# hzxie/Stereo-3D-Reconstruction

Measured on AMD Instinct MI355X. Metric: stereo pairs/s forward (batch 32, 224x224 -> 32^3 voxel), higher is better.
Workload: dtype f32

## Files before the change

stereo-3d-reconstruction_amd/csrc/s3r_api.hip:

```cpp
#include "s3r_host.h"

#include <algorithm>
#include <cmath>
#include <cstdio>
#include <cstring>
#include <utility>

using namespace s3rh;

namespace {

inline bool misaligned16(const void* p) { return ((uintptr_t)p & 15) != 0; }
int bf16_align_fail(const char* what, const void* p) {
    return fail(S3R_ERR_INVALID, "%s must be 16-byte aligned (got %p): bf16 tensors are accessed 16 bytes at a time", what, p);
}

struct ConvCall {
    const s3r_conv_desc* d;
    Geo g;
    const void* x; const void* x2; int nsplit, x_u8;
    const void* w; const float* scale; const float* shift;
    void* y;
    float* scratch; int64_t scratch_elems;
    hipStream_t s;
// ... 274 lines not shown
        return fail(S3R_ERR_INVALID, "a consumer's operand is written from the class-parallel launch form of a 3D two-axis layer only (the semi-fused "
                    "form of this batch keeps the plain output: s3r_chain_forward plans that itself)");
    if (g2.bmax <= 0 || ((pre || to_v || p.out_mode) && g2.bmax < d->batch))
        return fail(S3R_ERR_INVALID, "two-axis Winograd form: the transformed input of this batch exceeds 2 GiB (at most %d samples per "
                    "call with a producer-written input: s3r_conv_wino_input_elems)", g2.bmax);
    int rc = check_scratch(c, need.total, "the two-axis Winograd form of this layer needs");
    if (rc) return rc;
    p.w = c.wf() + packed_layout(d, g).wino2;
    p.x = pre ? c.xf() : c.scratch;
    p.part = c.scratch + need.v;
    p.Nd = g2.sg; p.Nh = g2.sg; p.Nw = g2.out;
    p.kd = 1; p.kh = 1; p.kw = g2.kw; p.T = g2.kw;
    p.x_hs = g2.wp; p.x_ds = g2.sg * g2.wp; p.x_cs = g2.sg * g2.sg * g2.wp;
    p.x_org = 0;
    set_divs(p);
    if (g2.ax == 2) {
        p.Nd = 1; p.Nw = g2.sg;
        p.dS = s3r::FastDiv((unsigned)(g2.sg * g2.sg));
        p.dW = s3r::FastDiv((unsigned)g2.sg);
    }
    p.Hout = g2.out; p.Dout = g2.out;
    p.ncls = g2.ncls;
    p.ksplit = 1;
    const int64_t x_sample = g.x_elems / d->batch;
    ps.launches = 0;
    for (int b0 = 0; b0 < d->batch; b0 += g2.bmax) {
        const int nb = sub_batch(d->batch, b0, g2.bmax);
        hipError_t e = hipSuccess;
        if (!pre) {
            s3r::AuxScope aux(c.s, 4.0 * ((double)nb * x_sample + (double)(g2.ax == 2 ? g2.ncls * d->cin * s3r::wino2_npad(g2.pos_sample * nb) : g2.v_sample * nb)));
            if (g2.ax == 2)
                e = s3r::launch_wino2p_input(c.xf() + (int64_t)b0 * x_sample, c.scratch, nb, d->cin, g2.wp, g2.wp, g2.sg, g2.sg,
                                             s3r::wino2_npad(g2.pos_sample * nb), c.s);
            else
                e = s3r::launch_wino2_input(c.xf() + (int64_t)b0 * x_sample, c.scratch, g2.ax, (long long)nb * d->cin, g2.wp, g2.wp, g2.wp, g2.sg,
                                            g2.sg, c.s);
            if (e != hipSuccess) return hip_fail(e, "two-axis Winograd input transform launch");
            ps.launches += 1;
        }
        set_sub_batch(p, c.yf(), b0, nb, g2.v_sample);
        p.x_cls = nb * d->cin * p.x_cs;
        int nl = 0;
        e = s3r::launch_conv_wino2(p, g2.ax, wino2_form_of(d, p.Ntotal, form), to_v, c.s, &nl);
        if (e != hipSuccess) return hip_fail(e, "two-axis Winograd conv launch");
        ps.launches += nl;
    }
// ... 1202 lines not shown
```

stereo-3d-reconstruction_amd/csrc/s3r_conv_wino.hip:

```cpp
#include "s3r_kernels.h"
#include <cstdlib>

namespace s3r {

typedef float wf32x16 __attribute__((ext_vector_type(16)));
typedef float wv2f __attribute__((ext_vector_type(2)));
template <int N> struct WVec;
template <> struct WVec<1> { typedef float type; };
template <> struct WVec<2> { typedef wv2f type; };
typedef float wv4f __attribute__((ext_vector_type(4)));
template <> struct WVec<4> { typedef wv4f type; };
template <int N>
__device__ __forceinline__ float wvget(const typename WVec<N>::type& v, int i) {
    if constexpr (N == 1) return v; else return v[i];
}

#define S3R_LDS_PTR_W(p) ((__attribute__((address_space(3))) void*)(p))

#ifndef S3R_WNB
#define S3R_WNB 2
#endif
#ifndef S3R_WBK
#define S3R_WBK 32
#endif
// ... 190 lines not shown
        y[3] = fmaf(8.f, d34, d12) + m[5];
    } else {
        const float t00 = m[0] + m[1], t01 = m[1] - m[2];
        const float t10 = m[3] + m[4], t11 = m[4] - m[5];
        const float t20 = m[6] + m[7], t21 = m[7] - m[8];
        y[0] = t00 + t10;
        y[1] = t01 + t11;
        y[2] = t10 - t20;
        y[3] = t11 - t21;
    }
}
template <int KIND>
__device__ __forceinline__ int wino_out_off(int i, int y_ds, int y_hs) {
    if constexpr (KIND == 1) return i * y_hs;
    else return (i >> 1) * 2 * y_ds + (i & 1) * 2 * y_hs;
}
__device__ __forceinline__ float wino_act(float y, float sc, float sf, float lo) { return fmaxf(fmaf(y, sc, sf), lo); }
__device__ __forceinline__ float wino_head_act(float t, int act) {
    if (act == ACT_RELU) return fmaxf(t, 0.f);
    if (act == ACT_SIGMOID) return __builtin_amdgcn_rcpf(1.f + __expf(-t));
    return t;
}

template <int VEC, int KIND, int WN, bool CP, bool HEAD, bool XM = false, bool SEMI = false>
__device__ __forceinline__ void wino_body(const ConvParams& p, const int bid_in, const int nwg_in, const int n_begin,
                                          const int n_end, float* __restrict__ wsmem) {
    constexpr bool DECONV = KIND == 2;
    constexpr int NCLS = WinoKind<KIND>::NCLS, R = WinoKind<KIND>::R;
    constexpr int WM = 4 / WN, TM = 2 / WM, BN = 32 * WN;
    constexpr int NACC = CP ? 1 : NCLS;
    static_assert(KIND == 1 || KIND == 2, "F(4,3) convolution or F(2,2) transposed convolution");
    static_assert(!SEMI || (KIND == 1 && !CP && !HEAD), "the semi-fused form: serial F(4,3) row classes of one depth class");
    static_assert(WN == 4 || WN == 2, "4 waves as 1 x 4 or 2 x 2");
    static_assert(!HEAD || (DECONV && !CP && WN == 2), "the fused head: serial transposed form");
    float* As = wsmem;
    constexpr int BSTG = (DECONV ? 2 : 1) * WBK * BN;
    float* Bs = wsmem + WNB * WBK * WBM;
    constexpr int PB = 64 * VEC;
    constexpr int NPIECE_B = WBK * BN / PB;
    static_assert(NPIECE_B % 4 == 0, "B pieces divide over the 4 waves");
    constexpr int NPB = NPIECE_B / 4;
    constexpr bool B_WIDE = BN >= PB;
    constexpr int PPR = B_WIDE ? BN / PB : 1;
    constexpr int RPP = B_WIDE ? 1 : PB / BN;
    constexpr int LPR_B = BN / VEC;
    constexpr int NPD = WNPA + NPB;

    const int tid = threadIdx.x;
    const int lane = tid & 63;
    const int wave = __builtin_amdgcn_readfirstlane(tid >> 6);
    const int wm = wave / WN, wn = wave % WN;
    const int j = lane & 31, h = lane >> 5;
#ifdef S3R_ABLATE
    unsigned long long tl0 = 0, tl1 = 0, tl2 = 0;
    if (p.debug == 7) tl0 = __builtin_amdgcn_s_memrealtime();
#endif

// ... 4 lines not shown
        const int q = nwg >> 3, r = nwg & 7, xcd = bid & 7, slot = bid >> 3;
        const int item = (xcd < r ? xcd * (q + 1) : r * (q + 1) + (xcd - r) * q) + slot;
        const int ntile = p.m_tiles * n_tiles;
        const int c = item / ntile;
        bid = item - c * ntile;
        if constexpr (DECONV) { pc = c / NCLS; cls0 = c - pc * NCLS; } else cls0 = SEMI ? c * NCLS : c;
    } else if constexpr (DECONV) {
        const int nwg = nwg_in >> 3;
        const int item = (bid & 7) * nwg + (bid >> 3);
        bid = item >> 3;
        pc = item & 7;
    } else {
        const int nwg = nwg_in;
        const int q = nwg >> 3, r = nwg & 7, xcd = bid & 7, slot = bid >> 3;
        bid = (xcd < r ? xcd * (q + 1) : r * (q + 1) + (xcd - r) * q) + slot;
    }
    const int rd = (pc >> 2) & 1, rh = (pc >> 1) & 1, rw = pc & 1;
    const int m_tile = bid % p.m_tiles, n_tile = bid / p.m_tiles;
    const int m0 = m_tile * WBM, n0 = n_begin + n_tile * BN;
    const int S = p.Nd * p.Nh * p.Nw;
    const int T = DECONV ? 2 : p.T;
    const int chunks = p.Cin / WBK;
    const int nkt = T * chunks;
    const int total = NACC * nkt;

    int bvoff;
    {
        int col, lrow;
        if (B_WIDE) { col = (wave % PPR) * PB + lane * VEC; lrow = 0; }
        else        { col = (lane % LPR_B) * VEC;           lrow = lane / LPR_B; }
        int n = n0 + col;
        if (n >= n_end) n = n_end - VEC;
        const int b = p.dS.div(n);
        int rem = n - b * S;
        const int pd = p.dHW.div(rem);
        rem -= pd * p.Nh * p.Nw;
        const int q = p.dW.div(rem);
        const int pw = rem - q * p.Nw;
        if constexpr (DECONV)
            bvoff = (b * p.Cin * p.x_cs + (2 * pd + rd) * p.x_ds + (2 * q + rh) * p.x_hs + pw + rw + lrow * p.x_cs) * 4;
        else
            bvoff = (b * p.Cin * p.x_cs + p.x_org + pd * p.x_ds + q * p.x_hs + pw + lrow * p.x_cs) * 4;
    }
    const int avoff = ((lane >> 4) * p.CoutPad + (lane & 15) * 4) * 4;
    const __amdgpu_buffer_rsrc_t xrsrc =
        __builtin_amdgcn_make_buffer_rsrc(const_cast<float*>(p.x), 0, (int)p.x_bytes, 0x00020000);
    const __amdgpu_buffer_rsrc_t drsrc =
        __builtin_amdgcn_make_buffer_rsrc(const_cast<float*>(DECONV ? p.xd : p.x), 0, (int)p.x_bytes, 0x00020000);
    const size_t x_el = (size_t)p.x_bytes / 4;
    const __amdgpu_buffer_rsrc_t wrsrc = __builtin_amdgcn_make_buffer_rsrc(
        const_cast<float*>(p.w), 0,
        (int)((unsigned)(DECONV ? 72 : (p.ncls ? p.ncls : NCLS)) * (unsigned)T * (unsigned)p.Cin * (unsigned)p.CoutPad * 4u),
        0x00020000);
    const int b_row0 = B_WIDE ? wave / PPR : wave * RPP;
    constexpr int B_ROW_STEP = B_WIDE ? 4 / PPR : 4 * RPP;
    const int b_lds0 = B_WIDE ? b_row0 * BN + (wave % PPR) * PB : wave * PB;
    constexpr int B_LDS_STEP = B_WIDE ? B_ROW_STEP * BN : 4 * PB;
    const int cs4 = p.x_cs * 4;

    int c_cls = cls0, c_cc = 0, c_td = 0, c_tw = 0, c_tap = 0;
    int c_kt = (DECONV ? pc * NCLS + cls0 : cls0) * nkt;
    int c_a = cls0 / 3, c_b = cls0 - 3 * (cls0 / 3);
#ifdef S3R_ABLATE
    bool abl_loop = false;
#endif
    auto issue = [&](int buf) __attribute__((always_inline)) {
#ifdef S3R_ABLATE
        const bool skip_a = abl_loop && (p.debug == 3 || p.debug == 5);
        const bool skip_b = abl_loop && (p.debug == 3 || p.debug == 4 || (p.debug == 6 && (DECONV ? c_tap != 0 : c_tw != 0)));
#else
        constexpr bool skip_a = false, skip_b = false;
#endif
        if (!skip_a) {
#pragma unroll
            for (int q = 0; q < WNPA; ++q)
                wdma<16>(wrsrc, As + buf * WBK * WBM + (wave + 4 * q) * 256, avoff,
                         (c_kt * WBK * p.CoutPad + m0) * 4 + (wave + 4 * q) * 4 * p.CoutPad * 4);
        }
        float* sb = Bs + buf * BSTG + b_lds0;
        if constexpr (DECONV) {
            const int b_base = ((c_cc * WBK + b_row0) * p.x_cs + (c_a ? p.x_ds : 0) + (c_b ? p.x_hs : 0) + c_tap) * 4;
            if (skip_b) {
            } else if constexpr (XM) {
                const int t_idx = (c_a != 1 ? 2 : 0) + (c_b != 1 ? 1 : 0);
                const float* tb = t_idx == 0 ? p.x : p.xd + (size_t)(t_idx - 1) * x_el;
                const __amdgpu_buffer_rsrc_t trsrc = __builtin_amdgcn_make_buffer_rsrc(const_cast<float*>(tb), 0, (int)p.x_bytes, 0x00020000);
#pragma unroll
                for (int q = 0; q < NPB; ++q) wdma<4 * VEC>(trsrc, sb + q * B_LDS_STEP, bvoff, b_base + q * B_ROW_STEP * cs4);
            } else if (c_b == 1) {
#pragma unroll
                for (int q = 0; q < NPB; ++q) wdma<4 * VEC>(xrsrc, sb + q * B_LDS_STEP, bvoff, b_base + q * B_ROW_STEP * cs4);
                if (c_a != 1) {
#pragma unroll
                    for (int q = 0; q < NPB; ++q)
                        wdma<4 * VEC>(xrsrc, sb + WBK * BN + q * B_LDS_STEP, bvoff, b_base + p.x_ds * 4 + q * B_ROW_STEP * cs4);
                }
            } else {
#pragma unroll
                for (int q = 0; q < NPB; ++q) wdma<4 * VEC>(drsrc, sb + q * B_LDS_STEP, bvoff, b_base + q * B_ROW_STEP * cs4);
                if (c_a != 1) {
#pragma unroll
                    for (int q = 0; q < NPB; ++q)
                        wdma<4 * VEC>(drsrc, sb + WBK * BN + q * B_LDS_STEP, bvoff, b_base + p.x_ds * 4 + q * B_ROW_STEP * cs4);
                }
            }
            ++c_kt;
            if (++c_tap == 2) {
                c_tap = 0;
                if (++c_cc == chunks) {
                    c_cc = 0; ++c_cls;
                    if (++c_b == 3) { c_b = 0; ++c_a; }
                }
            }
        } else {
            const int b_base = (c_cls * p.x_cls + (c_cc * WBK + b_row0) * p.x_cs + c_td * p.x_ds + c_tw) * 4;
            if (!skip_b) {
#pragma unroll
                for (int q = 0; q < NPB; ++q) wdma<4 * VEC>(xrsrc, sb + q * B_LDS_STEP, bvoff, b_base + q * B_ROW_STEP * cs4);
            }
            ++c_kt;
            if (++c_tw == p.kw) { c_tw = 0; ++c_td; }
            if (++c_tap == T) {
                c_tap = 0; c_td = 0; c_tw = 0;
                if (++c_cc == chunks) { c_cc = 0; ++c_cls; }
            }
        }
    };

    wf32x16 acc[NACC][TM];
#pragma unroll
    for (int c = 0; c < NACC; ++c)
#pragma unroll
        for (int t = 0; t < TM; ++t)
#pragma unroll
            for (int r = 0; r < 16; ++r) acc[c][t][r] = 0.f;

#pragma unroll
    for (int i = 0; i < WNB - 1; ++i)
        if (i < total) issue(i);
    if (total >= WNB - 1) asm volatile("s_waitcnt vmcnt(%0)" :: "n"((WNB - 2) * NPD) : "memory");
    else asm volatile("s_waitcnt vmcnt(0)" ::: "memory");
    __builtin_amdgcn_s_barrier();
    asm volatile("" ::: "memory");
#ifdef S3R_ABLATE
    abl_loop = true;
    if (p.debug == 7) tl1 = __builtin_amdgcn_s_memrealtime();
#endif

    const int a_off = h * WBM + wm * TM * 32 + j * TM;
    const int b_off = h * BN + wn * 32 + j;
    typedef typename WVec<TM>::type AV;
    int cur = 0, g = 0;
    auto run_class = [&](wf32x16 (&ac)[TM], const bool diff) __attribute__((always_inline)) {
        for (int kt = 0; kt < nkt; ++kt, ++g) {
            const bool more = g + WNB - 1 < total;
            if (more) issue(cur == 0 ? WNB - 1 : cur - 1);
            const float* a = As + cur * WBK * WBM + a_off;
            const float* b = Bs + cur * BSTG + b_off;
            if (DECONV && diff) {
#pragma unroll
                for (int ks = 0; ks < WBK / 2; ++ks) {
                    const AV av = *reinterpret_cast<const AV*>(a + ks * 2 * WBM);
                    const float bv = b[ks * 2 * BN] - b[WBK * BN + ks * 2 * BN];
#pragma unroll
                    for (int t = 0; t < TM; ++t) ac[t] = __builtin_amdgcn_mfma_f32_32x32x2f32(wvget<TM>(av, t), bv, ac[t], 0, 0, 0);
                }
            } else {
#pragma unroll
                for (int ks = 0; ks < WBK / 2; ++ks) {
                    const AV av = *reinterpret_cast<const AV*>(a + ks * 2 * WBM);
                    const float bv = b[ks * 2 * BN];
#pragma unroll
                    for (int t = 0; t < TM; ++t) ac[t] = __builtin_amdgcn_mfma_f32_32x32x2f32(wvget<TM>(av, t), bv, ac[t], 0, 0, 0);
                }
            }
            if (more) asm volatile("s_waitcnt vmcnt(%0)" :: "n"((WNB - 2) * NPD) : "memory");
            else asm volatile("s_waitcnt vmcnt(0)" ::: "memory");
// ... 153 lines not shown
                    const float sc = ep_sc[mbase + dm], sf = ep_sf[mbase + dm];
                    float m[NCLS], y[R];
#pragma unroll
                    for (int c = 0; c < NCLS; ++c) m[c] = acc[c][tm][r];
                    wino_out<KIND>(m, y);
                    const int so = dm * row_bytes;
                    if (ok) {
#pragma unroll
                        for (int i = 0; i < R; ++i)
                            if (i < row1) {
                                const float v = wino_act(y[i], sc, sf, lo);
                                __builtin_amdgcn_raw_buffer_store_b32(__builtin_bit_cast(unsigned, v), yrsrc,
                                                                      yvo0 + 4 * wino_out_off<KIND>(i, p.y_ds, p.y_hs), so, 0);
                            }
                    }
                    if ((r & 3) == 3) __builtin_amdgcn_sched_barrier(0);
                }
        }
        S3R_TL_FINISH();
    }
}
#undef S3R_TL_FINISH

template <int VEC, int KIND, int WN, bool CP, bool HEAD, bool XM = false, bool SEMI = false>
__global__ __launch_bounds__(256, (CP || KIND == 1 ? 4 : 3)) void wino_kernel(const ConvParams p) {
    extern __shared__ __attribute__((aligned(16))) float wsmem[];
    wino_body<VEC, KIND, WN, CP, HEAD, XM, SEMI>(p, blockIdx.x, gridDim.x, p.n_begin, p.n_end, wsmem);
}

template <int VEC, int KIND, bool HEAD = false, bool XM = false>
__global__ __launch_bounds__(256, (KIND == 1 ? 4 : 3)) void wino_dual_kernel(const ConvParams p) {
    extern __shared__ __attribute__((aligned(16))) float wsmem[];
    if ((int)blockIdx.x < p.big_wgs)
        wino_body<VEC, KIND, 2, false, HEAD, XM>(p, blockIdx.x, p.big_wgs, p.n_begin, p.n_cut, wsmem);
    else
        wino_body<VEC, KIND, 2, true, false, XM>(p, (int)blockIdx.x - p.big_wgs, (int)gridDim.x - p.big_wgs, p.n_cut, p.n_end, wsmem);
}

template <int KIND, bool HEAD>
__global__ __launch_bounds__(256) void wino_finish_kernel(const ConvParams p, const int n_begin, const int n_end, const int npad) {
    constexpr bool DECONV = KIND == 2;
    constexpr int NCLS = WinoKind<KIND>::NCLS, R = WinoKind<KIND>::R;
    const int S = p.Nd * p.Nh * p.Nw;
    const int nn = n_end - n_begin;
    const int pc = DECONV ? (int)blockIdx.y : 0;
    const int rd = (pc >> 2) & 1, rh = (pc >> 1) & 1, rw = pc & 1;
    const float lo = p.act == ACT_RELU ? 0.f : -__builtin_inff();
    constexpr int NBLK = DECONV ? 8 * NCLS : NCLS;
    const int ntl = npad >> 6;
    const float* __restrict__ base = p.part + (size_t)pc * NCLS * 64;
// ... 326 lines not shown
hipError_t launch_pack_wino2(const float* w, float* wp, int ax, int Cin, int Cout, int CoutPad, hipStream_t s) {
    if (ax == 0) hipLaunchKernelGGL(pack_wino2_kernel<0>, dim3(1024), dim3(256), 0, s, w, wp, Cin, Cout, CoutPad);
    else if (ax == 1) hipLaunchKernelGGL(pack_wino2_kernel<1>, dim3(1024), dim3(256), 0, s, w, wp, Cin, Cout, CoutPad);
    else if (ax == 2) hipLaunchKernelGGL(pack_wino2p_kernel, dim3(1024), dim3(256), 0, s, w, wp, Cin, Cout, CoutPad);
    else return hipErrorInvalidValue;
    return hipGetLastError();
}

__device__ __forceinline__ void wino2_copy_out(const float* __restrict__ lds, float* __restrict__ dst, int count, int tid) {
    if ((count & 3) == 0 && (reinterpret_cast<size_t>(dst) & 15) == 0) {
        for (int i = tid * 4; i < count; i += 1024) *reinterpret_cast<wv4f*>(dst + i) = *reinterpret_cast<const wv4f*>(lds + i);
    } else {
        for (int i = tid; i < count; i += 256) dst[i] = lds[i];
    }
}
__device__ __forceinline__ void wino2_zero_out(float* __restrict__ dst, int count, int tid) {
    if ((count & 3) == 0 && (reinterpret_cast<size_t>(dst) & 15) == 0) {
        for (int i = tid * 4; i < count; i += 1024) *reinterpret_cast<wv4f*>(dst + i) = wv4f{0.f, 0.f, 0.f, 0.f};
    } else {
        for (int i = tid; i < count; i += 256) dst[i] = 0.f;
    }
}

__global__ __launch_bounds__(256) void wino2s_finish_kernel(const ConvParams p, const int npad, const int halo, const int SUB,
                                                            const FastDiv dNd, const FastDiv dMS) {
    constexpr int N = 6, M = 4;
    extern __shared__ __attribute__((aligned(16))) float fsm[];
    const int tid = threadIdx.x;
    const int G = p.Nh * p.Nw, Wp = p.y_hs, slice = p.y_ds, MS = M * slice;
    const float lo = p.act == ACT_RELU ? 0.f : -__builtin_inff();
    const int per_c = p.B * p.Nd;
    const int nrg = (per_c + SUB - 1) / SUB;
    const bool vec = (slice & 3) == 0 && (reinterpret_cast<size_t>(p.y) & 15) == 0;
    for (int item = blockIdx.x; item < p.Cout * nrg; item += gridDim.x) {
        const int mrow = item / nrg;
        const int r0 = (item - mrow * nrg) * SUB;
        const int nsub = per_c - r0 < SUB ? per_c - r0 : SUB;
        for (int i = tid; i < nsub * MS; i += 256) fsm[i] = 0.f;
        __syncthreads();
        const float sc = p.scale ? p.scale[mrow] : 1.f, sf = p.shift ? p.shift[mrow] : 0.f;
        for (int t = tid; t < nsub * G; t += 256) {
            const int sub = p.dHW.div(t);
            const int g = t - sub * G;
            const int sh = p.dW.div(g);
            const int pw = g - sh * p.Nw;
            const int r = r0 + sub;
            const int sd = r - dNd.div(r) * p.Nd;
            const int n = r0 * G + t;
            const float* __restrict__ src = p.part + ((size_t)mrow * (npad >> 6) + (n >> 6)) * (N * M * 64) + (n & 63);
            float* __restrict__ o = fsm + sub * MS + (halo + M * sh) * Wp + halo + pw;
#pragma unroll
            for (int v = 0; v < M; ++v) {
                float m[N], y[M];
#pragma unroll
                for (int a = 0; a < N; ++a) m[a] = src[(a * M + v) * 64];
                wax_at<0>(m, y);
#pragma unroll
                for (int u = 0; u < M; ++u)
                    if (M * sd + u < p.Dout && M * sh + v < p.Hout) o[u * slice + v * Wp] = wino_act(y[u], sc, sf, lo);
            }
        }
        __syncthreads();
        float* __restrict__ yc = p.y + (size_t)mrow * p.y_cs;
        for (int e = vec ? tid * 4 : tid; e < nsub * MS; e += vec ? 1024 : 256) {
            const int sub = dMS.div(e);
            const int off = e - sub * MS;
            const int r = r0 + sub;
            const int b = dNd.div(r);
// ... 10 lines not shown
                const int b = dNd.div(r);
                const int sd = r - b * p.Nd;
                if (sd == 0) wino2_zero_out(yc + (size_t)b * p.y_bs, halo * slice, tid);
                if (sd == p.Nd - 1) wino2_zero_out(yc + (size_t)b * p.y_bs + (size_t)(halo + p.Dout) * slice, halo * slice, tid);
            }
        __syncthreads();
    }
}

template <int AX>
__global__ __launch_bounds__(256) void wino2_finish_flat_kernel(const ConvParams p, const int npad) {
    constexpr int N = WAxis<AX>::N, M = WAxis<AX>::M;
    const int S = p.Nd * p.Nh * p.Nw;
    const int nn = p.Ntotal;
    const float lo = p.act == ACT_RELU ? 0.f : -__builtin_inff();
    const long long total = (long long)p.Cout * nn;
    for (long long i = (long long)blockIdx.x * 256 + threadIdx.x; i < total; i += (long long)gridDim.x * 256) {
        const int mrow = (int)(i / nn);
        const int n = (int)(i - (long long)mrow * nn);
        const int b = p.dS.div(n);
        int rem = n - b * S;
        const int sd = p.dHW.div(rem);
        rem -= sd * p.Nh * p.Nw;
        const int sh = p.dW.div(rem);
        const int pw = rem - sh * p.Nw;
        const float* __restrict__ src = p.part + ((size_t)mrow * (npad >> 6) + (n >> 6)) * (N * N * 64) + (n & 63);
        float t[N][M];
#pragma unroll
        for (int a = 0; a < N; ++a) {
            float m[N], y[M];
#pragma unroll
            for (int c = 0; c < N; ++c) m[c] = src[(a * N + c) * 64];
            wax_at<AX>(m, y);
#pragma unroll
            for (int v = 0; v < M; ++v) t[a][v] = y[v];
        }
        const float sc = p.scale ? p.scale[mrow] : 1.f, sf = p.shift ? p.shift[mrow] : 0.f;
        float* __restrict__ yo = p.y + (size_t)b * p.y_bs + (size_t)mrow * p.y_cs + p.y_org + (size_t)M * sd * p.y_ds + M * sh * p.y_hs + pw;
#pragma unroll
        for (int v = 0; v < M; ++v) {
            float m[N], y[M];
#pragma unroll
            for (int a = 0; a < N; ++a) m[a] = t[a][v];
            wax_at<AX>(m, y);
#pragma unroll
            for (int u = 0; u < M; ++u)
                if (M * sd + u < p.Dout && M * sh + v < p.Hout) yo[(size_t)u * p.y_ds + v * p.y_hs] = wino_act(y[u], sc, sf, lo);
        }
// ... 222 lines not shown
    const int S = p.Nd * p.Nh * p.Nw;
    const int G1 = PROD == 2 ? 8 * S : S;
    const int G2 = CONS == 2 ? vol : SG * SG * Op;
    const int ncb = (p.Cout + CB - 1) / CB;
    const float lo = p.act == ACT_RELU ? 0.f : -__builtin_inff();
    const bool vec2 = CONS == 2 && (Op & 1) == 0 && (reinterpret_cast<size_t>(p.y) & 7) == 0;
    for (int item = blockIdx.x; item < p.B * ncb; item += gridDim.x) {
        const int b = item / ncb;
        const int c0 = (item - b * ncb) * CB;
        const int nc = p.Cout - c0 < CB ? p.Cout - c0 : CB;
        for (int i = tid; i < nc * vol; i += 256) hsm[i] = 0.f;
        __syncthreads();
        for (int t = tid; t < nc * G1; t += 256) {
            const int cl = dG1.div(t);
            int g = t - cl * G1;
            const int mrow = c0 + cl;
            const float sc = p.scale ? p.scale[mrow] : 1.f, sf = p.shift ? p.shift[mrow] : 0.f;
            float* __restrict__ o = hsm + cl * vol + org;
            if constexpr (PROD <= 1) {
                constexpr int N = WAxis<PROD>::N, M = WAxis<PROD>::M;
                const int n = b * S + g;
                const int sd = p.dHW.div(g);
                g -= sd * p.Nh * p.Nw;
                const int sh = p.dW.div(g);
                const int pw = g - sh * p.Nw;
                const float* __restrict__ src = p.part + ((size_t)mrow * (npad >> 6) + (n >> 6)) * (N * N * 64) + (n & 63);
                float tt[N][M];
#pragma unroll
                for (int a = 0; a < N; ++a) {
                    float m[N], y[M];
#pragma unroll
                    for (int c = 0; c < N; ++c) m[c] = src[(a * N + c) * 64];
                    wax_at<PROD>(m, y);
#pragma unroll
                    for (int v = 0; v < M; ++v) tt[a][v] = y[v];
                }
                o += M * sd * ds + M * sh * hs + pw;
#pragma unroll
                for (int v = 0; v < M; ++v) {
                    float m[N], y[M];
#pragma unroll
                    for (int a = 0; a < N; ++a) m[a] = tt[a][v];
                    wax_at<PROD>(m, y);
#pragma unroll
                    for (int u = 0; u < M; ++u)
                        if (M * sd + u < p.Dout && M * sh + v < p.Hout) o[u * ds + v * hs] = wino_act(y[u], sc, sf, lo);
                }
            } else if constexpr (PROD == 2) {
// ... 196 lines not shown
        q.dS = q.dHW = q.dW = FastDiv((unsigned)npad);
        q.kd = q.kh = q.kw = 1; q.T = 1;
        q.x_org = 0; q.x_ds = 0; q.x_hs = 0; q.x_cs = npad; q.x_cls = p.Cin * npad;
        q.x_bytes = (unsigned)(4ull * 36 * p.Cin * npad);
        q.Ntotal = npad; q.n_end = npad;
        const dim3 grid(p.m_tiles * n_tiles * (form == 1 ? 6 : 36));
        if (form == 1) hipLaunchKernelGGL((wino_kernel<4, 1, 2, false, false, false, true>), grid, dim3(256), lds, stream, q);
        else hipLaunchKernelGGL((wino_kernel<4, 1, 2, true, false>), grid, dim3(256), lds, stream, q);
        hipError_t e = hipGetLastError();
        if (e != hipSuccess) return e;
        const long long items = (long long)p.Cout * ((p.B + PL - 1) / PL);
        const dim3 fgrid((unsigned)(items < 16384 ? items : 16384));
        const size_t flds = (size_t)PL * plane * 4;
        AuxScope aux(stream, 4.0 * (double)p.Cout * ((double)(form == 1 ? 24 : 36) * npad + (to_v ? 36.0 * npad : (double)p.B * plane)));
        if (to_v) {
            if (form == 1) hipLaunchKernelGGL((wino2p_finish_kernel<true, true>), fgrid, dim3(256), flds, stream, p, npad, halo, PL);
            else hipLaunchKernelGGL((wino2p_finish_kernel<false, true>), fgrid, dim3(256), flds, stream, p, npad, halo, PL);
        } else if (form == 1) hipLaunchKernelGGL((wino2p_finish_kernel<true, false>), fgrid, dim3(256), flds, stream, p, npad, halo, PL);
        else hipLaunchKernelGGL((wino2p_finish_kernel<false, false>), fgrid, dim3(256), flds, stream, p, npad, halo, PL);
        if (launches) *launches = 2;
        return hipGetLastError();
    }
    if (p.y_ds != p.y_hs * p.y_hs || p.y_cs != (p.Dout + 2 * halo) * p.y_ds) return hipErrorInvalidValue;
    if (form == 1) {
        const int M = wino2_outputs(ax), G = p.Nh * p.Nw;
        if (ax != 0 || (size_t)M * p.y_ds * 4 > 64 * 1024) return hipErrorInvalidValue;
        int SUB = 256 / G < 1 ? 1 : 256 / G;
        if (SUB > p.B * p.Nd) SUB = p.B * p.Nd;
        while (SUB > 1 && (size_t)SUB * M * p.y_ds * 4 > 64 * 1024) --SUB;
        const size_t flds = (size_t)SUB * M * p.y_ds * 4;
        const FastDiv dNd((unsigned)p.Nd), dMS((unsigned)(M * p.y_ds));
        const long long items = (long long)p.Cout * ((p.B * p.Nd + SUB - 1) / SUB);
        const dim3 fgrid((unsigned)(items < 32768 ? items : 32768));
        const dim3 grid(p.m_tiles * n_tiles * 6);
        if (p.Nw % 4 == 0) hipLaunchKernelGGL((wino_kernel<4, 1, 2, false, false, false, true>), grid, dim3(256), lds, stream, p);
        else hipLaunchKernelGGL((wino_kernel<1, 1, 2, false, false, false, true>), grid, dim3(256), lds, stream, p);
        hipError_t e = hipGetLastError();
        if (e != hipSuccess) return e;
        AuxScope aux(stream, 4.0 * (double)p.Cout * (24.0 * n_tiles * WCN + (double)p.B * p.y_cs));
        hipLaunchKernelGGL(wino2s_finish_kernel, fgrid, dim3(256), flds, stream, p, n_tiles * WCN, halo, SUB, dNd, dMS);
        if (launches) *launches = 2;
        return hipGetLastError();
    }
    const dim3 grid(p.m_tiles * n_tiles * p.ncls);
    if (p.Nw % 4 == 0) hipLaunchKernelGGL((wino_kernel<4, 1, 2, true, false>), grid, dim3(256), lds, stream, p);
    else hipLaunchKernelGGL((wino_kernel<1, 1, 2, true, false>), grid, dim3(256), lds, stream, p);
    hipError_t e = hipGetLastError();
    if (e != hipSuccess) return e;
    if (launches) *launches = 2;
    if (p.out_mode) return launch_wino_handoff(p, ax, p.out_mode - 1, n_tiles * WCN, stream);
    const long long total = (long long)p.Cout * p.Ntotal;
    const long long blocks = (total + 255) / 256;
    const dim3 flat((unsigned)(blocks < 8192 ? blocks : 8192));
    AuxScope aux(stream, 4.0 * (double)p.Cout * ((double)p.ncls * n_tiles * WCN + (double)p.B * p.Dout * p.Hout * p.Nw));
    if (ax == 0) hipLaunchKernelGGL(wino2_finish_flat_kernel<0>, flat, dim3(256), 0, stream, p, n_tiles * WCN);
    else hipLaunchKernelGGL(wino2_finish_flat_kernel<1>, flat, dim3(256), 0, stream, p, n_tiles * WCN);
    if (launches) *launches = 2;
    return hipGetLastError();
}

#ifdef S3R_ABLATE
}
extern "C" int s3r_debug_read_timeline_wino(unsigned long long* out, int nblocks) {
    if (nblocks > 65536) nblocks = 65536;
    return hipMemcpyFromSymbol(out, HIP_SYMBOL(s3r::s3r_wino_timeline), sizeof(unsigned long long) * 6 * (size_t)nblocks) == hipSuccess ? nblocks : -1;
}
extern "C" int s3r_debug_clear_timeline_wino() {
    void* ptr = nullptr;
    if (hipGetSymbolAddress(&ptr, HIP_SYMBOL(s3r::s3r_wino_timeline)) != hipSuccess) return -1;
// ... 7 lines not shown
```

stereo-3d-reconstruction_amd/csrc/s3r_kernels.h:

```cpp
#pragma once
#include <hip/hip_runtime.h>
#include <stdint.h>
#include <atomic>

struct s3r_optim_tensor;
struct s3r_augment_desc;

namespace s3r {

struct LdsAttr {
    std::atomic<unsigned long long> done{0};
    hipError_t ensure(const void* fn, int bytes) {
        int dev = 0;
        hipError_t e = hipGetDevice(&dev);
        if (e != hipSuccess) return e;
        if (dev >= 0 && dev < 64 && ((done.load(std::memory_order_relaxed) >> dev) & 1ull)) return hipSuccess;
        e = hipFuncSetAttribute(fn, hipFuncAttributeMaxDynamicSharedMemorySize, bytes);
        if (e == hipSuccess && dev >= 0 && dev < 64) done.fetch_or(1ull << dev, std::memory_order_relaxed);
        return e;
    }
};

inline int cu_count() {
    static std::atomic<int> cached[64];
// ... 58 lines not shown
    int y_step;
    int shuf_s, shuf_nd;
    FastDiv dSC, dS1;
    unsigned x_bytes;
    unsigned y_bytes;
    int transposed;
    int act;
    float slope;
    int Ntotal;
    int n_begin, n_end;
    int n_tiles, m_tiles;
    int n_cut, big_wgs;
    int ksplit;
    float* part;
    int debug;
    const float* head_w;
    const float* head_scale;
    const float* head_shift;
    int head_act;
    int x_cls, Hout, Dout, ncls;
    const float* xd;
    int xd_mode;
    int out_mode;
};

struct TClsEntry {
    int Nd, Nh, Nw, kd, kh, kw, T, x_org, y_org, Ntotal, wg_begin, w_off;
    FastDiv dS, dHW, dW;
};
constexpr int kTClsMax = 27;
struct TClsTable { int n; TClsEntry e[kTClsMax]; };
hipError_t launch_conv_tcls(const ConvParams& base, TClsTable tab, hipStream_t stream);

enum { WINO_SERIAL = 0, WINO_CP = 1, WINO_DUAL = 2 };
struct WinoLaunch { int mode, n_cut; };

struct ConvParamsH {
    const void* x;
    const void* w;
    const float* scale;
    const float* shift;
    void* y;
    float* part;
    int B, Cin, Cout, CoutPad;
    int Nd, Nh, Nw;
    FastDiv dS, dHW, dW, dDH, dH;
// ... 190 lines not shown
```

stereo-3d-reconstruction_amd/csrc/s3r_pointwise.hip:

```cpp
#include "s3r_kernels.h"

namespace s3r {

typedef float v4f __attribute__((ext_vector_type(4)));

__device__ __forceinline__ float apply_act(float v, int act) {
    if (act == ACT_RELU) return fmaxf(v, 0.f);
    if (act == ACT_SIGMOID) return 1.f / (1.f + __expf(-v));
    return v;
}

template <typename TI>
__global__ __launch_bounds__(256) void stem_kernel(const TI* __restrict__ x, const TI* __restrict__ x2, int nsplit,
                                                   const float* __restrict__ wt,
                                                   const float* __restrict__ scale, const float* __restrict__ shift,
                                                   float* __restrict__ y, int N, int Hi, int Wi, int Ho, int Wo,
                                                   int y_cs, int y_hs, int y_org) {
    const int HWo = Ho * Wo;
    const long long total = (long long)N * HWo;
    const long long gid = (long long)blockIdx.x * 256 + threadIdx.x;
    if (gid >= total) return;
    const int n = (int)(gid / HWo);
    const int sp = (int)(gid - (long long)n * HWo);
    const int oh = sp / Wo, ow = sp - oh * Wo;
// ... 300 lines not shown
    float* sl = cvw2_smem;
    float* sr = cvw2_smem + HW;
    const int bc = blockIdx.x;
    const int b = bc / C, c = bc - b * C;
    const float* __restrict__ pl = fl + (size_t)bc * HW;
    const float* __restrict__ pr = fr + (size_t)bc * HW;
    for (int i = threadIdx.x; i < HW; i += 256) {
        sl[i] = pl[i];
        sr[i] = pr[i];
    }
    __syncthreads();
    const int Wp = W + 2, SH = H / 4, SD = (D + 3) / 4;
    const int ds = SH * Wp;
    const int run = SD * ds;
    const int ny = (int)gridDim.y, pph = ny > 1 ? ny / 2 : 1;
    const int half0 = ny > 1 ? (int)blockIdx.y / pph : 0, half1 = ny > 1 ? half0 + 1 : 2;
    const int part = ny > 1 ? (int)blockIdx.y - half0 * pph : 0;
    const int e0 = (part * SD / pph) * ds, e1 = ((part + 1) * SD / pph) * ds;
    for (int half = half0; half < half1; ++half) {
        float* __restrict__ o = V + ((size_t)b * 2 * C + half * C + c) * run;
        for (int e = e0 + threadIdx.x; e < e1; e += 256) {
            const int sd = dPlane.div(e);
            const int rem = e - sd * ds;
            const int sh = dRow.div(rem);
            const int wp = rem - sh * Wp;
            const int w = wp - 1;
            float t[6][6];
#pragma unroll
            for (int a = 0; a < 6; ++a) {
                const int d = 4 * sd + a - 1;
                float r[6], v[6];
#pragma unroll
                for (int k = 0; k < 6; ++k) {
                    const int h = 4 * sh + k - 1;
                    const bool in = (unsigned)d < (unsigned)D && (unsigned)h < (unsigned)H && (unsigned)w < (unsigned)W;
                    const int hw = h * W + w;
                    r[k] = half == 0 ? ((in && w >= d) ? sl[hw] - sr[hw - d] : 0.f) : ((in && w + d < W) ? sr[hw] - sl[hw + d] : 0.f);
                }
                wino_rows_to_classes<4>(r, v);
#pragma unroll
                for (int k = 0; k < 6; ++k) t[a][k] = v[k];
            }
#pragma unroll
            for (int k = 0; k < 6; ++k) {
                float r[6], v[6];
#pragma unroll
                for (int a = 0; a < 6; ++a) r[a] = t[a][k];
                wino_rows_to_classes<4>(r, v);
#pragma unroll
                for (int a = 0; a < 6; ++a) o[e + (size_t)(a * 6 + k) * cls_stride] = v[a];
            }
        }
    }
}

hipError_t launch_cost_volume_wino2(const float* fl, const float* fr, float* V, int B, int C, int D, int H, int W, hipStream_t s) {
    const size_t lds = (size_t)2 * H * W * sizeof(float);
    const int Wp = W + 2, SH = H / 4, SD = (D + 3) / 4;
    const long long cls_stride = (long long)B * 2 * C * SD * SH * Wp;
    const int ny = B * C <= 128 ? 2 * SD : B * C <= 512 ? 2 : 1;
    hipLaunchKernelGGL(cost_volume_wino2_kernel, dim3(B * C, ny), dim3(256), lds, s, fl, fr, V, C, D, H, W, cls_stride,
                       FastDiv((unsigned)(SH * Wp)), FastDiv((unsigned)Wp));
    return hipGetLastError();
}

hipError_t launch_cost_volume(const float* fl, const float* fr, float* vol, int B, int C, int D, int H, int W,
                              int halo, hipStream_t s) {
    const size_t lds = (size_t)2 * H * W * sizeof(float);
    const int Wp = W + 2 * halo, Hp = H + 2 * halo;
    hipLaunchKernelGGL(cost_volume_kernel, dim3(B * C), dim3(256), lds, s, fl, fr, vol, C, D, H, W, halo,
                       FastDiv((unsigned)(Hp * Wp)), FastDiv((unsigned)Wp));
    return hipGetLastError();
}

__global__ __launch_bounds__(256) void pad_copy_kernel(const float* __restrict__ x, float* __restrict__ y,
                                                       long long total, int D, int H, int W, int hd, int hh, int hw) {
    const int Hp = H + 2 * hh, Wp = W + 2 * hw;
    const long long Dp = D + 2 * hd;
    for (long long i = (long long)blockIdx.x * 256 + threadIdx.x; i < total; i += (long long)gridDim.x * 256) {
        const int w = (int)(i % W);
        long long r = i / W;
        const int h = (int)(r % H);
        r /= H;
        const int d = (int)(r % D);
        const long long pl = r / D;
// ... 441 lines not shown
```

stereo-3d-reconstruction_amd/modules.py:

```python
from __future__ import annotations

import ctypes as C
import dataclasses
import os
from typing import Dict, Optional, Sequence

import torch
import torch.nn as nn

from . import _lib
from . import arch_spec as spec
from ._tensors import _check_input, _check_input_cl, _check_render, _stream_ptr, _to_logical, channels_last_to_f32
from .ops import (_StemFunction, differentiable_batchnorm, differentiable_conv, differentiable_cost_volume, differentiable_disparity_soft,
                  differentiable_head, differentiable_linear, disparity_soft, disparity_wta)

MAX_CHUNK = 256

_DEBUG = {"tile": {}, "ksplit": {}, "algo": {}}


class debug_overrides:

    def __init__(self, tile=None, ksplit=None, algo=None):
        self._new = {"tile": dict(tile or {}), "ksplit": dict(ksplit or {}), "algo": dict(algo or {})}
# ... 429 lines not shown
        if B == 0:
            return vol
        _lib.check(_lib.load().s3r_cost_volume_forward(fl.data_ptr(), fr.data_ptr(), vol.data_ptr(), B, Cc,
                                                       self.max_disp, H, W, halo, _stream_ptr(fl.device)),
                   "cost_volume")
        return vol

    @torch.no_grad()
    def forward_wino(self, feat_left: torch.Tensor, feat_right: torch.Tensor) -> torch.Tensor:
        fl = _check_input(feat_left, "feat_left", feat_left.shape[1:])
        fr = _check_input(feat_right, "feat_right", feat_left.shape[1:])
        B, Cc, H, W = fl.shape
        shape = (6, B, 2 * Cc, self.max_disp + 2, H // 4, W + 2)
        planes = self._resident("_planes", shape, fl.device)
        _lib.check(_lib.load().s3r_cost_volume_forward_wino(fl.data_ptr(), fr.data_ptr(), planes.data_ptr(), B, Cc,
                                                            self.max_disp, H, W, _stream_ptr(fl.device)), "cost_volume (wino)")
        return planes

    @torch.no_grad()
    def forward_wino2(self, feat_left: torch.Tensor, feat_right: torch.Tensor) -> torch.Tensor:
        fl = _check_input(feat_left, "feat_left", feat_left.shape[1:])
        fr = _check_input(feat_right, "feat_right", feat_left.shape[1:])
        B, Cc, H, W = fl.shape
        shape = (36, B, 2 * Cc, self.max_disp // 4, H // 4, W + 2)
        planes = self._resident("_planes", shape, fl.device)
        _lib.check(_lib.load().s3r_cost_volume_forward_wino2(fl.data_ptr(), fr.data_ptr(), planes.data_ptr(), B, Cc,
                                                             self.max_disp, H, W, _stream_ptr(fl.device)), "cost_volume (wino2)")
        return planes

    def forward_for(self, consumer, feat_left: torch.Tensor, feat_right: torch.Tensor):
        layout = consumer.wino_input_layout(feat_left.shape[0])
        if layout == _lib.LAYOUT_WINO_H:
            return self.forward_wino(feat_left, feat_right), layout
        if layout == _lib.LAYOUT_WINO_DH:
            return self.forward_wino2(feat_left, feat_right), layout
        return self.forward_padded(feat_left, feat_right), _lib.LAYOUT_PLAIN

    @torch.no_grad()
    def forward(self, feat_left: torch.Tensor, feat_right: torch.Tensor) -> torch.Tensor:
        if self.precision == "bf16":
            return _to_logical(self._bf16(feat_left, feat_right, 0, resident=False))
        if feat_left.shape != feat_right.shape or feat_left.dim() != 4:
            raise RuntimeError(f"feature maps must both be (B,C,H,W), got {tuple(feat_left.shape)} and "
                               f"{tuple(feat_right.shape)}")
        fl = _check_input(feat_left, "feat_left", feat_left.shape[1:])
        fr = _check_input(feat_right, "feat_right", feat_left.shape[1:])
        B, Cc, H, W = fl.shape
        vol = torch.empty((B, 2 * Cc, self.max_disp, H, W), dtype=torch.float32, device=fl.device)
        if B == 0:
            return vol
        _lib.check(_lib.load().s3r_cost_volume_forward(fl.data_ptr(), fr.data_ptr(), vol.data_ptr(), B, Cc,
                                                       self.max_disp, H, W, 0, _stream_ptr(fl.device)), "cost_volume")
        return vol

    def differentiable(self, feat_left: torch.Tensor, feat_right: torch.Tensor) -> torch.Tensor:
        _fp32_only(self, "CostVolume.differentiable", "the cost-volume backward kernel reads fp32 tensors")
        return differentiable_cost_volume(feat_left, feat_right, self.max_disp)


def _check_wino_planes(v: torch.Tensor, layout: int = _lib.LAYOUT_WINO_H) -> torch.Tensor:
    if layout == _lib.LAYOUT_WINO_DH:
        ncls, want = 36, (2 * spec.FEAT_C, spec.MAX_DISP // 4, spec.FEAT_HW // 4, spec.FEAT_HW + 2)
    else:
        ncls, want = 6, (2 * spec.FEAT_C, spec.MAX_DISP + 2, spec.FEAT_HW // 4, spec.FEAT_HW + 2)
    if not isinstance(v, torch.Tensor) or not v.is_cuda or v.dtype != torch.float32 or v.dim() != 6 or v.shape[0] != ncls or \
            tuple(v.shape[2:]) != want or not v.is_contiguous():
        raise RuntimeError(f"transformed volume must be a contiguous float32 HIP tensor ({ncls}, B, {', '.join(map(str, want))})")
    return v


class _VolumeChain(_HipChain):
    _entry = "s3r_decoder_forward"

    def __init__(self, layers, precision: str, winograd):
        super().__init__(layers, spec.MAX_DISP, tag_base=200, precision=precision, winograd=winograd)

    def _run_plain(self, volume: torch.Tensor, upto: Optional[str] = None) -> torch.Tensor:
        tail = (2 * spec.FEAT_C, spec.MAX_DISP, spec.FEAT_HW, spec.FEAT_HW)
        check = _check_input_cl if self.precision == "bf16" else _check_input
        return self._run(check(volume, "volume", tail), upto)

    def _run_padded(self, volume_padded: torch.Tensor, halo: int, in_layout: int, upto: Optional[str] = None) -> torch.Tensor:
        if in_layout in (_lib.LAYOUT_WINO_H, _lib.LAYOUT_WINO_DH):
            return self._run(_check_wino_planes(volume_padded, in_layout), upto, in_halo=1, in_layout=in_layout)
        n = (spec.MAX_DISP + 2 * halo, spec.FEAT_HW + 2 * halo, spec.FEAT_HW + 2 * halo)
        if self.precision == "bf16":
            x = _check_input(volume_padded, "volume_padded", n + (2 * spec.FEAT_C,), torch.bfloat16)
        else:
            x = _check_input(volume_padded, "volume_padded", (2 * spec.FEAT_C,) + n)
        return self._run(x, upto, in_halo=halo)
# ... 239 lines not shown
```

Baseline: 8847.

## Skip dead cost-volume K tiles in two-axis Winograd consumer via transposed plane layout

The cost volume's two-axis Winograd planes are now stored with the width and row axes swapped. The first decoder convolution uses a new live-K-tile path that works out, per output tile, which channel-half and tap chunks of the cost volume are structurally zero at low disparities. It iterates only over the live tiles using a bitmask, which cuts MFMA work and loads for blocks that cover zero regions. In exchange the kernel gets an extra template variant, the finish kernels and Python validation must handle the new layout, and there are tight preconditions (a 32-bit live mask and fixed shape relations).

```diff
diff --git a/stereo-3d-reconstruction_amd/csrc/s3r_api.hip b/stereo-3d-reconstruction_amd/csrc/s3r_api.hip
--- a/stereo-3d-reconstruction_amd/csrc/s3r_api.hip
+++ b/stereo-3d-reconstruction_amd/csrc/s3r_api.hip
@@ -320,6 +320,7 @@
     p.Hout = g2.out; p.Dout = g2.out;
     p.ncls = g2.ncls;
     p.ksplit = 1;
+    p.cv_n = d->in_layout == S3R_LAYOUT_WINO_DH ? g2.out : 0;
     const int64_t x_sample = g.x_elems / d->batch;
     ps.launches = 0;
     for (int b0 = 0; b0 < d->batch; b0 += g2.bmax) {
diff --git a/stereo-3d-reconstruction_amd/csrc/s3r_conv_wino.hip b/stereo-3d-reconstruction_amd/csrc/s3r_conv_wino.hip
--- a/stereo-3d-reconstruction_amd/csrc/s3r_conv_wino.hip
+++ b/stereo-3d-reconstruction_amd/csrc/s3r_conv_wino.hip
@@ -1,4 +1,5 @@
 #include "s3r_kernels.h"
+#include "s3r_cv_live.h"
 #include <cstdlib>
 
 namespace s3r {
@@ -236,7 +237,7 @@
     return t;
 }
 
-template <int VEC, int KIND, int WN, bool CP, bool HEAD, bool XM = false, bool SEMI = false>
+template <int VEC, int KIND, int WN, bool CP, bool HEAD, bool XM = false, bool SEMI = false, bool CVL = false>
 __device__ __forceinline__ void wino_body(const ConvParams& p, const int bid_in, const int nwg_in, const int n_begin,
                                           const int n_end, float* __restrict__ wsmem) {
     constexpr bool DECONV = KIND == 2;
@@ -247,6 +248,7 @@
     static_assert(!SEMI || (KIND == 1 && !CP && !HEAD), "the semi-fused form: serial F(4,3) row classes of one depth class");
     static_assert(WN == 4 || WN == 2, "4 waves as 1 x 4 or 2 x 2");
     static_assert(!HEAD || (DECONV && !CP && WN == 2), "the fused head: serial transposed form");
+    static_assert(!CVL || (KIND == 1 && (CP || SEMI)), "live K tiles: the two-axis forms of the cost volume's consumer");
     float* As = wsmem;
     constexpr int BSTG = (DECONV ? 2 : 1) * WBK * BN;
     float* Bs = wsmem + WNB * WBK * WBM;
@@ -297,7 +299,22 @@
     const int T = DECONV ? 2 : p.T;
     const int chunks = p.Cin / WBK;
     const int nkt = T * chunks;
-    const int total = NACC * nkt;
+    int nrun = nkt;
+    unsigned live = 0;
+    if constexpr (CVL) {
+        const int last = (n0 + BN < n_end ? n0 + BN : n_end) - 1, half_c = p.Cin >> 1;
+        const int g = p.dW.div(n0), sd = g - p.dNh.div(g) * p.Nh;
+        const bool one = p.dW.div(last) == g;
+        const int w_lo = p.dNh.div(n0 - g * p.Nw), w_hi = p.dNh.div(last - g * p.Nw);
+        for (int tw = 0; tw < 3; ++tw) {
+            const bool l0 = !s3r_cv_ktile_dead_at(p.cv_n, 0, tw, one, sd, w_lo, w_hi);
+            const bool l1 = !s3r_cv_ktile_dead_at(p.cv_n, 1, tw, one, sd, w_lo, w_hi);
+            for (int cc = 0; cc < chunks; ++cc)
+                if ((cc * WBK < half_c && l0) || (cc * WBK + WBK > half_c && l1)) live |= 1u << (cc * 3 + tw);
+        }
+        nrun = __builtin_popcount(live);
+    }
+    const int total = NACC * nrun;
 
     int bvoff;
     {
@@ -336,6 +353,7 @@
     int c_cls = cls0, c_cc = 0, c_td = 0, c_tw = 0, c_tap = 0;
     int c_kt = (DECONV ? pc * NCLS + cls0 : cls0) * nkt;
     int c_a = cls0 / 3, c_b = cls0 - 3 * (cls0 / 3);
+    unsigned c_rem = live;
 #ifdef S3R_ABLATE
     bool abl_loop = false;
 #endif
@@ -346,6 +364,10 @@
 #else
         constexpr bool skip_a = false, skip_b = false;
 #endif
+        if constexpr (CVL) {
+            c_tap = __builtin_ctz(c_rem);
+            c_kt = c_cls * nkt + c_tap;
+        }
         if (!skip_a) {
 #pragma unroll
             for (int q = 0; q < WNPA; ++q)
@@ -387,6 +409,15 @@
                     if (++c_b == 3) { c_b = 0; ++c_a; }
                 }
             }
+        } else if constexpr (CVL) {
+            const int cc = c_tap / 3;
+            const int b_base = (c_cls * p.x_cls + (cc * WBK + b_row0) * p.x_cs + (c_tap - 3 * cc) * p.x_ds) * 4;
+            if (!skip_b) {
+#pragma unroll
+                for (int q = 0; q < NPB; ++q) wdma<4 * VEC>(xrsrc, sb + q * B_LDS_STEP, bvoff, b_base + q * B_ROW_STEP * cs4);
+            }
+            c_rem &= c_rem - 1;
+            if (c_rem == 0) { c_rem = live; ++c_cls; }
         } else {
             const int b_base = (c_cls * p.x_cls + (c_cc * WBK + b_row0) * p.x_cs + c_td * p.x_ds + c_tw) * 4;
             if (!skip_b) {
@@ -427,7 +458,7 @@
     typedef typename WVec<TM>::type AV;
     int cur = 0, g = 0;
     auto run_class = [&](wf32x16 (&ac)[TM], const bool diff) __attribute__((always_inline)) {
-        for (int kt = 0; kt < nkt; ++kt, ++g) {
+        for (int kt = 0; kt < nrun; ++kt, ++g) {
             const bool more = g + WNB - 1 < total;
             if (more) issue(cur == 0 ? WNB - 1 : cur - 1);
             const float* a = As + cur * WBK * WBM + a_off;
@@ -627,10 +658,10 @@
 }
 #undef S3R_TL_FINISH
 
-template <int VEC, int KIND, int WN, bool CP, bool HEAD, bool XM = false, bool SEMI = false>
+template <int VEC, int KIND, int WN, bool CP, bool HEAD, bool XM = false, bool SEMI = false, bool CVL = false>
 __global__ __launch_bounds__(256, (CP || KIND == 1 ? 4 : 3)) void wino_kernel(const ConvParams p) {
     extern __shared__ __attribute__((aligned(16))) float wsmem[];
-    wino_body<VEC, KIND, WN, CP, HEAD, XM, SEMI>(p, blockIdx.x, gridDim.x, p.n_begin, p.n_end, wsmem);
+    wino_body<VEC, KIND, WN, CP, HEAD, XM, SEMI, CVL>(p, blockIdx.x, gridDim.x, p.n_begin, p.n_end, wsmem);
 }
 
 template <int VEC, int KIND, bool HEAD = false, bool XM = false>
@@ -1003,6 +1034,11 @@
     }
 }
 
+__device__ __forceinline__ void wino2_group_pos(const ConvParams& p, int g, int& sh, int& pw) {
+    if (p.cv_n) { pw = p.dNh.div(g); sh = g - pw * p.Nh; }
+    else { sh = p.dW.div(g); pw = g - sh * p.Nw; }
+}
+
 __global__ __launch_bounds__(256) void wino2s_finish_kernel(const ConvParams p, const int npad, const int halo, const int SUB,
                                                             const FastDiv dNd, const FastDiv dMS) {
     constexpr int N = 6, M = 4;
@@ -1023,8 +1059,8 @@
         for (int t = tid; t < nsub * G; t += 256) {
             const int sub = p.dHW.div(t);
             const int g = t - sub * G;
-            const int sh = p.dW.div(g);
-            const int pw = g - sh * p.Nw;
+            int sh, pw;
+            wino2_group_pos(p, g, sh, pw);
             const int r = r0 + sub;
             const int sd = r - dNd.div(r) * p.Nd;
             const int n = r0 * G + t;
@@ -1081,8 +1117,8 @@
         int rem = n - b * S;
         const int sd = p.dHW.div(rem);
         rem -= sd * p.Nh * p.Nw;
-        const int sh = p.dW.div(rem);
-        const int pw = rem - sh * p.Nw;
+        int sh, pw;
+        wino2_group_pos(p, rem, sh, pw);
         const float* __restrict__ src = p.part + ((size_t)mrow * (npad >> 6) + (n >> 6)) * (N * N * 64) + (n & 63);
         float t[N][M];
 #pragma unroll
@@ -1351,8 +1387,8 @@
                 const int n = b * S + g;
                 const int sd = p.dHW.div(g);
                 g -= sd * p.Nh * p.Nw;
-                const int sh = p.dW.div(g);
-                const int pw = g - sh * p.Nw;
+                int sh, pw;
+                wino2_group_pos(p, g, sh, pw);
                 const float* __restrict__ src = p.part + ((size_t)mrow * (npad >> 6) + (n >> 6)) * (N * N * 64) + (n & 63);
                 float tt[N][M];
 #pragma unroll
@@ -1595,6 +1631,17 @@
         return hipGetLastError();
     }
     if (p.y_ds != p.y_hs * p.y_hs || p.y_cs != (p.Dout + 2 * halo) * p.y_ds) return hipErrorInvalidValue;
+    ConvParams q = p;
+    const bool cvl = p.cv_n > 0;
+    if (cvl) {
+        if (ax != 0 || p.kw != 3 || p.Nw != p.cv_n || p.Nh * 4 != p.cv_n || p.Nd != p.Nh || (p.Cin & 1)) return hipErrorInvalidValue;
+        q.Nd = 1; q.Nh = p.Nd; q.Nw = p.Nw * p.Nh;
+        q.dS = q.dHW = FastDiv((unsigned)(q.Nh * q.Nw)); q.dW = FastDiv((unsigned)q.Nw);
+        q.kd = 3; q.kw = 1; q.T = 3;
+        q.x_hs = p.x_hs * p.Nh; q.x_ds = p.Nh;
+        p.dNh = q.dNh = FastDiv((unsigned)p.Nh);
+    }
+    const bool cvl_skip = cvl && 3 * (p.Cin / WBK) <= 32;
     if (form == 1) {
         const int M = wino2_outputs(ax), G = p.Nh * p.Nw;
         if (ax != 0 || (size_t)M * p.y_ds * 4 > 64 * 1024) return hipErrorInvalidValue;
@@ -1606,8 +1653,9 @@
         const long long items = (long long)p.Cout * ((p.B * p.Nd + SUB - 1) / SUB);
         const dim3 fgrid((unsigned)(items < 32768 ? items : 32768));
         const dim3 grid(p.m_tiles * n_tiles * 6);
-        if (p.Nw % 4 == 0) hipLaunchKernelGGL((wino_kernel<4, 1, 2, false, false, false, true>), grid, dim3(256), lds, stream, p);
-        else hipLaunchKernelGGL((wino_kernel<1, 1, 2, false, false, false, true>), grid, dim3(256), lds, stream, p);
+        if (cvl_skip) hipLaunchKernelGGL((wino_kernel<4, 1, 2, false, false, false, true, true>), grid, dim3(256), lds, stream, q);
+        else if (q.Nw % 4 == 0) hipLaunchKernelGGL((wino_kernel<4, 1, 2, false, false, false, true>), grid, dim3(256), lds, stream, q);
+        else hipLaunchKernelGGL((wino_kernel<1, 1, 2, false, false, false, true>), grid, dim3(256), lds, stream, q);
         hipError_t e = hipGetLastError();
         if (e != hipSuccess) return e;
         AuxScope aux(stream, 4.0 * (double)p.Cout * (24.0 * n_tiles * WCN + (double)p.B * p.y_cs));
@@ -1616,8 +1664,9 @@
         return hipGetLastError();
     }
     const dim3 grid(p.m_tiles * n_tiles * p.ncls);
-    if (p.Nw % 4 == 0) hipLaunchKernelGGL((wino_kernel<4, 1, 2, true, false>), grid, dim3(256), lds, stream, p);
-    else hipLaunchKernelGGL((wino_kernel<1, 1, 2, true, false>), grid, dim3(256), lds, stream, p);
+    if (cvl_skip) hipLaunchKernelGGL((wino_kernel<4, 1, 2, true, false, false, false, true>), grid, dim3(256), lds, stream, q);
+    else if (q.Nw % 4 == 0) hipLaunchKernelGGL((wino_kernel<4, 1, 2, true, false>), grid, dim3(256), lds, stream, q);
+    else hipLaunchKernelGGL((wino_kernel<1, 1, 2, true, false>), grid, dim3(256), lds, stream, q);
     hipError_t e = hipGetLastError();
     if (e != hipSuccess) return e;
     if (launches) *launches = 2;
diff --git a/stereo-3d-reconstruction_amd/csrc/s3r_cv_live.h b/stereo-3d-reconstruction_amd/csrc/s3r_cv_live.h
--- /dev/null
+++ b/stereo-3d-reconstruction_amd/csrc/s3r_cv_live.h
@@ -0,0 +1,22 @@
+#ifndef S3R_CV_LIVE_H
+#define S3R_CV_LIVE_H
+
+#if defined(__HIPCC__)
+#define S3R_CV_HD __host__ __device__ __forceinline__
+#else
+#define S3R_CV_HD static inline
+#endif
+
+S3R_CV_HD int s3r_cv_ktile_dead_at(int n, int half, int tw, int one_group, int sd, int w_lo, int w_hi) {
+    if (!one_group || sd < 1) return 0;
+    if (half == 0) return w_hi + tw < 4 * sd;
+    return w_lo + tw - 1 >= n + 1 - 4 * sd;
+}
+
+S3R_CV_HD int s3r_cv_ktile_dead(int n, int half, int tw, int first, int last, int per_group, int groups, int rows) {
+    const int g = first / per_group;
+    const int r0 = first - g * per_group, r1 = last - g * per_group;
+    return s3r_cv_ktile_dead_at(n, half, tw, last / per_group == g, g % groups, r0 / rows, r1 / rows);
+}
+
+#endif
diff --git a/stereo-3d-reconstruction_amd/csrc/s3r_kernels.h b/stereo-3d-reconstruction_amd/csrc/s3r_kernels.h
--- a/stereo-3d-reconstruction_amd/csrc/s3r_kernels.h
+++ b/stereo-3d-reconstruction_amd/csrc/s3r_kernels.h
@@ -104,6 +104,8 @@
     const float* xd;
     int xd_mode;
     int out_mode;
+    int cv_n;
+    FastDiv dNh;
 };
 
 struct TClsEntry {
diff --git a/stereo-3d-reconstruction_amd/csrc/s3r_pointwise.hip b/stereo-3d-reconstruction_amd/csrc/s3r_pointwise.hip
--- a/stereo-3d-reconstruction_amd/csrc/s3r_pointwise.hip
+++ b/stereo-3d-reconstruction_amd/csrc/s3r_pointwise.hip
@@ -346,8 +346,8 @@
         for (int e = e0 + threadIdx.x; e < e1; e += 256) {
             const int sd = dPlane.div(e);
             const int rem = e - sd * ds;
-            const int sh = dRow.div(rem);
-            const int wp = rem - sh * Wp;
+            const int wp = dRow.div(rem);
+            const int sh = rem - wp * SH;
             const int w = wp - 1;
             float t[6][6];
 #pragma unroll
@@ -384,7 +384,7 @@
     const long long cls_stride = (long long)B * 2 * C * SD * SH * Wp;
     const int ny = B * C <= 128 ? 2 * SD : B * C <= 512 ? 2 : 1;
     hipLaunchKernelGGL(cost_volume_wino2_kernel, dim3(B * C, ny), dim3(256), lds, s, fl, fr, V, C, D, H, W, cls_stride,
-                       FastDiv((unsigned)(SH * Wp)), FastDiv((unsigned)Wp));
+                       FastDiv((unsigned)(SH * Wp)), FastDiv((unsigned)SH));
     return hipGetLastError();
 }
 
diff --git a/stereo-3d-reconstruction_amd/modules.py b/stereo-3d-reconstruction_amd/modules.py
--- a/stereo-3d-reconstruction_amd/modules.py
+++ b/stereo-3d-reconstruction_amd/modules.py
@@ -475,11 +475,11 @@
         fl = _check_input(feat_left, "feat_left", feat_left.shape[1:])
         fr = _check_input(feat_right, "feat_right", feat_left.shape[1:])
         B, Cc, H, W = fl.shape
-        shape = (36, B, 2 * Cc, self.max_disp // 4, H // 4, W + 2)
+        shape = (36, B, 2 * Cc, self.max_disp // 4, W + 2, H // 4)
         planes = self._resident("_planes", shape, fl.device)
         _lib.check(_lib.load().s3r_cost_volume_forward_wino2(fl.data_ptr(), fr.data_ptr(), planes.data_ptr(), B, Cc,
                                                              self.max_disp, H, W, _stream_ptr(fl.device)), "cost_volume (wino2)")
-        return planes
+        return planes.transpose(-1, -2)
 
     def forward_for(self, consumer, feat_left: torch.Tensor, feat_right: torch.Tensor):
         layout = consumer.wino_input_layout(feat_left.shape[0])
@@ -517,8 +517,11 @@
     else:
         ncls, want = 6, (2 * spec.FEAT_C, spec.MAX_DISP + 2, spec.FEAT_HW // 4, spec.FEAT_HW + 2)
     if not isinstance(v, torch.Tensor) or not v.is_cuda or v.dtype != torch.float32 or v.dim() != 6 or v.shape[0] != ncls or \
-            tuple(v.shape[2:]) != want or not v.is_contiguous():
+            tuple(v.shape[2:]) != want or (layout != _lib.LAYOUT_WINO_DH and not v.is_contiguous()):
         raise RuntimeError(f"transformed volume must be a contiguous float32 HIP tensor ({ncls}, B, {', '.join(map(str, want))})")
+    if layout == _lib.LAYOUT_WINO_DH:
+        phys = v.transpose(-1, -2)
+        return (phys if phys.is_contiguous() else phys.contiguous()).transpose(-1, -2)
     return v
 
 
```

Result: faster. 8946 (median of 6 runs) (+1.1%).
